# liyi14/mx-DeepIM

Measured on NVIDIA H100. Metric: 480x640 4-iter pose refinements/sec, higher is better.
Workload: dtype fp16

## Files before the change

mx-deepim_b200/csrc/conv_igemm.cuh:

```cuda
#pragma once
#include <cuda.h>
#include <cuda_fp16.h>
#include "common.cuh"
#include "wgmma.cuh"

namespace dim {

struct ConvKParams {
  CUtensorMap a_map[4];
  CUtensorMap a_lo_map[4];
  CUtensorMap b_map;
  CUtensorMap b_lo_map;
  CUtensorMap out_map[2];
  const __nv_bfloat16 *in_hi, *in_lo;
  int in_cols;
  int KH, KW, stride, cchunks;
  int BW, BH, n_col_tiles;
  int Hq, Ho, Wo, Bn;
  int out_Hp, out_Wp, out_py, out_px, Cout;
  int kblocks;
  float slope;
  const float *bias;
  __nv_bfloat16 *out_hi, *out_lo;
  int in_off_r, in_off_c;
// ... 127 lines not shown
}

__device__ __forceinline__ uint32_t pack2_f16(float a, float b) {
  uint32_t r;
  asm("cvt.rn.satfinite.f16x2.f32 %0, %1, %2;" : "=r"(r) : "f"(b), "f"(a));
  return r;
}
__device__ __forceinline__ uint32_t pack2_bf16(float a, float b) {
  uint32_t r;
  asm("cvt.rn.bf16x2.f32 %0, %1, %2;" : "=r"(r) : "f"(b), "f"(a));
  return r;
}

constexpr int kConv1Slack = 2048;


__device__ __forceinline__ int frag_row(int t) { return ((t >> 5) << 4) + ((t & 31) >> 2); }

__device__ __forceinline__ uint32_t pack2_bf16_lo(float v0, float v1, uint32_t hi) {
  return pack2_bf16(v0 - __uint_as_float(hi << 16), v1 - __uint_as_float(hi & 0xFFFF0000u));
}

template <bool SPLIT3, bool F16>
__device__ __forceinline__ void epi_pack(float v0, float v1, float b0, float b1, float slope, uint32_t &hi, uint32_t &lo) {
  v0 += b0;
  v1 += b1;
  v0 = v0 > 0.f ? v0 : v0 * slope;
  v1 = v1 > 0.f ? v1 : v1 * slope;
  if (F16) {
    hi = pack2_f16(v0, v1);
  } else {
    hi = pack2_bf16(v0, v1);
    if (SPLIT3) lo = pack2_bf16_lo(v0, v1, hi);
  }
}

template <bool SPLIT3, bool F16>
__device__ __forceinline__ void store_pair(float v0, float v1, float2 b, float slope, __nv_bfloat16 *out_hi, __nv_bfloat16 *out_lo,
                                           long long off) {
  uint32_t h, l = 0;
  epi_pack<SPLIT3, F16>(v0, v1, b.x, b.y, slope, h, l);
  *reinterpret_cast<uint32_t *>(out_hi + off) = h;
  if (SPLIT3) *reinterpret_cast<uint32_t *>(out_lo + off) = l;
}

template <bool SPLIT3>
__device__ __forceinline__ void store_pair_generic(float v0, float v1, const ConvKParams &p, int n, bool valid, long long off,
                                                   long long add_off, long long mask_off) {
  if (!valid || n >= p.Cout) return;
  if (p.bias) {
    v0 += __ldg(p.bias + n);
    v1 += __ldg(p.bias + n + 1);
  }
  if (p.addend.p) {
    const __nv_bfloat162 a = *reinterpret_cast<const __nv_bfloat162 *>(p.addend.p + add_off);
    if (SPLIT3) {
      const __nv_bfloat162 al = *reinterpret_cast<const __nv_bfloat162 *>(p.addend.lo + add_off);
      v0 += __low2float(a) + __low2float(al);
      v1 += __high2float(a) + __high2float(al);
    } else {
      v0 += __low2float(a);
      v1 += __high2float(a);
    }
  }
  if (p.mask.p) {
    if (n < p.mask_climit) {
      const __nv_bfloat162 m = *reinterpret_cast<const __nv_bfloat162 *>(p.mask.p + mask_off);
      if (!(__low2float(m) > 0.f)) v0 *= p.slope;
      if (!(__high2float(m) > 0.f)) v1 *= p.slope;
    }
  } else {
    v0 = v0 > 0.f ? v0 : v0 * p.slope;
    v1 = v1 > 0.f ? v1 : v1 * p.slope;
  }
  if (SPLIT3) {
    const uint32_t h = pack2_bf16(v0, v1);
    *reinterpret_cast<uint32_t *>(p.out_hi + off) = h;
    *reinterpret_cast<uint32_t *>(p.out_lo + off) = pack2_bf16_lo(v0, v1, h);
  } else {
    *reinterpret_cast<__nv_bfloat162 *>(p.out_hi + off) = __floats2bfloat162_rn(v0, v1);
  }
}

template <int BLOCK_N, int STAGES, bool SPLIT3, int EPI>
struct ConvSmem2 {
  static constexpr int A_BYTES = 128 * 64 * 2;
  static constexpr int B_BYTES = BLOCK_N * 64 * 2;
  static constexpr int NPREC = SPLIT3 ? 2 : 1;
  static constexpr int STAGE_BYTES = (A_BYTES + B_BYTES) * NPREC;
  static constexpr int RING_BYTES = STAGES * STAGE_BYTES;
  static constexpr int LIMIT = 227 * 1024, FIXED = 1024  + 256 ;
  static constexpr bool TMA_EPI = EPI == 0 && !SPLIT3;
  static constexpr int STG_GROUPS =
      !TMA_EPI ? 0 : (RING_BYTES + 2 * BLOCK_N * 128 + FIXED <= LIMIT ? BLOCK_N / 64 : BLOCK_N / 128);
  static constexpr int STG_ROUNDS = TMA_EPI ? BLOCK_N / 64 / STG_GROUPS : 0;
  static constexpr int STG_BYTES = STG_GROUPS * 8192;
  static constexpr int TOTAL = RING_BYTES + 2 * STG_BYTES + FIXED;
  static_assert(TOTAL <= LIMIT, "conv_igemm shared memory");
};

template <int BLOCK_N, int STAGES, bool SPLIT3, bool F16, int EPI = 0>
__global__ void __launch_bounds__(384, 1) conv_igemm_persistent_kernel(const __grid_constant__ ConvKParams p,
                                                                       const int total_tiles, const int n_tiles) {
  using S = ConvSmem2<BLOCK_N, STAGES, SPLIT3, EPI>;
  constexpr uint32_t SBO = 1024u;

  extern __shared__ uint8_t smem_raw[];
  uint8_t *smem = reinterpret_cast<uint8_t *>((reinterpret_cast<uintptr_t>(smem_raw) + 1023) & ~(uintptr_t)1023);
  uint8_t *stg = smem + S::RING_BYTES;
  uint64_t *full_bar = reinterpret_cast<uint64_t *>(stg + 2 * S::STG_BYTES);
  uint64_t *empty_bar = full_bar + STAGES;

  const int wgi = threadIdx.x >> 7, warp = threadIdx.x >> 5;

  if (threadIdx.x == 0) {
    for (int s = 0; s < STAGES; ++s) {
      ptx::mbar_init(&full_bar[s], 1);
      ptx::mbar_init(&empty_bar[s], 2);
    }
    ptx::fence_barrier_init();
    ptx::prefetch_tmap(&p.b_map);
    ptx::prefetch_tmap(&p.a_map[0]);
    if (S::TMA_EPI) ptx::prefetch_tmap(&p.out_map[0]);
  }
  __syncthreads();

  if (wgi == 0) {
    ptx::regs_producer();
    if (warp == 0) {
      const uint32_t tx = (uint32_t)(p.BW * p.BH * 64 * 2 + BLOCK_N * 64 * 2) * S::NPREC;
      int s = 0;
      uint32_t ph = 0;
      for (int tile = blockIdx.x; tile < total_tiles; tile += gridDim.x) {
        const int nt = tile % n_tiles, mt = tile / n_tiles;
        const int col_tile = mt % p.n_col_tiles, row_tile = mt / p.n_col_tiles;
        const int g0 = row_tile * p.BH, ow0 = col_tile * p.BW, n0 = nt * BLOCK_N;
        for (int kb = 0; kb < p.kblocks; ++kb) {
          ptx::mbar_wait(&empty_bar[s], ph ^ 1u);
          const int tap = kb / p.cchunks, cc = kb - tap * p.cchunks;
          const int kh = tap / p.KW, kw = tap - kh * p.KW;
          int view = 0, dr = kh, dc = kw;
          if (p.stride == 2) {
            view = ((kh & 1) << 1) | (kw & 1);
            dr = kh >> 1;
            dc = kw >> 1;
          }
          uint8_t *st = smem + s * S::STAGE_BYTES;
          if (EPI) { dr += p.in_off_r; dc += p.in_off_c; }
          if (ptx::elect_one()) {
            ptx::mbar_expect_tx_raw(&full_bar[s], tx);
            for (int pr = 0; pr < S::NPREC; ++pr) {
              uint8_t *sa = st + pr * (S::A_BYTES + S::B_BYTES);
              const CUtensorMap *am = pr ? &p.a_lo_map[view] : &p.a_map[view];
              ptx::tma_load_3d_raw(sa, am, &full_bar[s], cc * 64, ow0 + dc, g0 + dr);
              if (EPI == 0) ptx::tma_load_3d_raw(sa + S::A_BYTES / 2, am, &full_bar[s], cc * 64, ow0 + dc, g0 + dr + (p.BH >> 1));
              ptx::tma_load_2d_raw(sa + S::A_BYTES, pr ? &p.b_lo_map : &p.b_map, &full_bar[s], kb * 64, n0);
            }
          }
          __syncwarp();
          if (++s == STAGES) { s = 0; ph ^= 1u; }
        }
      }
    }
  } else {
    ptx::regs_consumer();
    const int t = threadIdx.x & 127;
    const int half = wgi - 1;
    const int q2 = (t & 3) * 2;
    const bool arriver = t == 0;
    const uint32_t base = ptx::smem_u32(smem);
    uint8_t *my_stg = stg + half * S::STG_BYTES;
    const int lane = t & 31;
    const uint32_t st_addr = ptx::smem_u32(my_stg) + (uint32_t)((16 * (t >> 5) + 8 * ((lane >> 3) & 1) + (lane & 7)) * 128);
    const uint32_t st_sw = (uint32_t)(((lane >> 4) & 1) ^ (lane & 7));
    float acc[BLOCK_N / 2];
    int s = 0;
    uint32_t ph = 0;
    for (int tile = blockIdx.x; tile < total_tiles; tile += gridDim.x) {
      int prev = -1;
      for (int kb = 0; kb < p.kblocks; ++kb) {
        ptx::mbar_wait(&full_bar[s], ph);
        const uint32_t a_hi = base + s * S::STAGE_BYTES + half * 8192;
        const uint32_t b_hi = base + s * S::STAGE_BYTES + S::A_BYTES;
        const uint64_t da0 = ptx::gmma_desc(a_hi, 16, SBO, ptx::kSW128), db0 = ptx::gmma_desc(b_hi, 16, SBO, ptx::kSW128);
        const uint64_t dal0 = da0 + ((S::A_BYTES + S::B_BYTES) >> 4), dbl0 = db0 + ((S::A_BYTES + S::B_BYTES) >> 4);
        wg::fence_acc(acc);
        wg::fence();
#pragma unroll
        for (int k = 0; k < 4; ++k) {
          const uint64_t da = da0 + (uint64_t)(2 * k), db = db0 + (uint64_t)(2 * k);
          wg::mma<BLOCK_N, F16, 0, 0>(acc, da, db, (kb > 0 || k > 0) ? 1u : 0u);
          if (SPLIT3) {
            wg::mma<BLOCK_N, false, 0, 0>(acc, dal0 + (uint64_t)(2 * k), db, 1u);
            wg::mma<BLOCK_N, false, 0, 0>(acc, da, dbl0 + (uint64_t)(2 * k), 1u);
          }
        }
        wg::commit();
        wg::wait<1>();
        wg::fence_acc(acc);
        if (prev >= 0 && arriver) ptx::mbar_arrive(&empty_bar[prev]);
        prev = s;
        if (++s == STAGES) { s = 0; ph ^= 1u; }
      }
      wg::wait<0>();
      wg::fence_acc(acc);
      if (prev >= 0 && arriver) ptx::mbar_arrive(&empty_bar[prev]);

      const int nt = tile % n_tiles, mt = tile / n_tiles;
      const int col_tile = mt % p.n_col_tiles, row_tile = mt / p.n_col_tiles;
      const int n0 = nt * BLOCK_N;
      if constexpr (S::TMA_EPI) {
        const int gs = row_tile * p.BH + half * (p.BH >> 1), ow0 = col_tile * p.BW;
        const int n_img = gs / p.Hq, oh = gs - n_img * p.Hq;
        const bool store0 = n_img < p.Bn && oh < p.Ho, store1 = n_img + 1 < p.Bn && oh + (p.BH >> 1) > p.Hq;
#pragma unroll
        for (int rd = 0; rd < S::STG_ROUNDS; ++rd) {
          if (arriver) ptx::bulk_wait_read0();
          ptx::named_bar_sync(1 + half, 128);
#pragma unroll
          for (int i = 0; i < S::STG_GROUPS * 4; ++i) {
            const int j = rd * S::STG_GROUPS * 8 + 2 * i;
            const float *bj = p.bias + n0 + 8 * j + q2;
            const float b0 = __ldg(bj), b1 = __ldg(bj + 1), b2 = __ldg(bj + 8), b3 = __ldg(bj + 9);
            uint32_t h[4], unused;
            epi_pack<false, F16>(acc[4 * j + 0], acc[4 * j + 1], b0, b1, p.slope, h[0], unused);
            epi_pack<false, F16>(acc[4 * j + 2], acc[4 * j + 3], b0, b1, p.slope, h[1], unused);
            epi_pack<false, F16>(acc[4 * j + 4], acc[4 * j + 5], b2, b3, p.slope, h[2], unused);
            epi_pack<false, F16>(acc[4 * j + 6], acc[4 * j + 7], b2, b3, p.slope, h[3], unused);
            ptx::stmatrix_x4(st_addr + (uint32_t)((i >> 2) * 8192) + (((uint32_t)(2 * (i & 3)) ^ st_sw) << 4), h);
          }
          ptx::fence_proxy_async();
          ptx::named_bar_sync(1 + half, 128);
          if (arriver && store0) {
            for (int q = 0; q < S::STG_GROUPS; ++q)
              ptx::tma_store_4d(&p.out_map[0], my_stg + q * 8192, n0 + (rd * S::STG_GROUPS + q) * 64, ow0, oh, n_img);
            ptx::bulk_commit();
          }
        }
        if (store1) {
#pragma unroll
          for (int rr = 0; rr < 2; ++rr) {
            const int lr = frag_row(t) + rr * 8, bh = lr / p.BW;
            const int oh1 = oh + bh - p.Hq, ow = ow0 + lr - bh * p.BW;
            if (lr < p.BW * (p.BH >> 1) && oh1 >= 0 && oh1 < p.Ho) {
              const long long off =
                  (((long long)(n_img + 1) * p.out_Hp + oh1 + p.out_py) * p.out_Wp + ow + p.out_px) * p.Cout + n0 + q2;
#pragma unroll
              for (int j = 0; j < BLOCK_N / 8; ++j)
                store_pair<false, F16>(acc[4 * j + 2 * rr], acc[4 * j + 2 * rr + 1],
                                       make_float2(__ldg(p.bias + n0 + 8 * j + q2), __ldg(p.bias + n0 + 8 * j + q2 + 1)), p.slope,
                                       p.out_hi, p.out_lo, off + 8 * j);
            }
          }
        }
      } else {
#pragma unroll
        for (int rr = 0; rr < 2; ++rr) {
          const int lr = frag_row(t) + rr * 8, m = EPI ? half * 64 + lr : lr;
          const bool in_tile = EPI ? m < p.BW * p.BH : lr < p.BW * (p.BH >> 1);
          const int bh = m / p.BW, bw = m - bh * p.BW;
          const int g = row_tile * p.BH + (EPI ? 0 : half * (p.BH >> 1)) + bh, ow = col_tile * p.BW + bw;
          const int n_img = g / p.Hq, oh = g - n_img * p.Hq;
          if (EPI == 1) {
            const int y = oh * p.out_sy + p.out_oy, x = ow * p.out_sx + p.out_ox;
            const bool valid = in_tile && (n_img < p.Bn) && (oh < p.Ho) && (ow < p.Wo) && y >= 0 && y < p.out_H &&
                               x >= 0 && x < p.out_W;
            const long long off =
                (((long long)n_img * p.out_Hp + y + p.out_py) * p.out_Wp + x + p.out_px) * p.out_cs + p.out_coff + n0 + q2;
            const long long add_off =
                (((long long)n_img * p.addend.Hp + y + p.addend.py) * p.addend.Wp + x + p.addend.px) * p.addend.cs + p.addend.coff +
                n0 + q2;
            const long long mask_off =
                (((long long)n_img * p.mask.Hp + y + p.mask.py) * p.mask.Wp + x + p.mask.px) * p.mask.cs + p.mask.coff + n0 + q2;
#pragma unroll
            for (int j = 0; j < BLOCK_N / 8; ++j)
              store_pair_generic<SPLIT3>(acc[4 * j + 2 * rr], acc[4 * j + 2 * rr + 1], p, n0 + 8 * j + q2, valid, off + 8 * j,
                                 add_off + 8 * j, mask_off + 8 * j);
          } else {
            const bool valid = in_tile && (n_img < p.Bn) && (oh < p.Ho) && (ow < p.Wo);
            if (valid) {
              const long long off = (((long long)n_img * p.out_Hp + oh + p.out_py) * p.out_Wp + ow + p.out_px) * p.Cout + n0 + q2;
#pragma unroll
              for (int j = 0; j < BLOCK_N / 8; ++j)
                store_pair<SPLIT3, F16>(acc[4 * j + 2 * rr], acc[4 * j + 2 * rr + 1],
                                        make_float2(__ldg(p.bias + n0 + 8 * j + q2), __ldg(p.bias + n0 + 8 * j + q2 + 1)), p.slope, p.out_hi,
                                        p.out_lo, off + 8 * j);
            }
          }
        }
      }
    }
    if (S::TMA_EPI && arriver) ptx::bulk_wait0();
  }
}

constexpr int kConv1StoreN = 80;

template <int N, int STAGES, bool SPLIT3>
struct Conv1Smem {
  static constexpr int NPREC = SPLIT3 ? 2 : 1;
  static constexpr int TAP_BYTES = 64 * 32 * 2;
  static constexpr int RES_BYTES = 16 * TAP_BYTES * NPREC;
  static constexpr int STG_BYTES = N * 128;
  static constexpr int PLANE_BYTES = (N + 3) * 16;
  static constexpr int STRIP_BYTES = (4 * PLANE_BYTES + 127) / 128 * 128;
  static constexpr int STAGE_BYTES = STRIP_BYTES * NPREC;
  static constexpr int TOTAL = RES_BYTES + 2 * STG_BYTES * NPREC + STAGES * STAGE_BYTES + 1024  + 256 ;
  static_assert(N % kConv1StoreN == 0 && N % 16 == 0 && STG_BYTES % 1024 == 0, "conv1 tile width");
  static_assert(TOTAL <= 227 * 1024, "conv1 shared memory");
};

template <int N, int STAGES, bool SPLIT3, bool F16>
__global__ void __launch_bounds__(384, 1) conv1_kernel(const __grid_constant__ ConvKParams p, const int rows_total,
                                                       const int rows_per_chunk, const int chunks_per_col) {
  using S = Conv1Smem<N, STAGES, SPLIT3>;
  extern __shared__ uint8_t smem_raw[];
  uint8_t *smem = reinterpret_cast<uint8_t *>((reinterpret_cast<uintptr_t>(smem_raw) + 1023) & ~(uintptr_t)1023);
  uint8_t *res = smem;
  uint8_t *stg = res + S::RES_BYTES;
  uint8_t *ring = stg + 2 * S::NPREC * S::STG_BYTES;
  uint64_t *full_bar = reinterpret_cast<uint64_t *>(ring + STAGES * S::STAGE_BYTES);
  uint64_t *empty_bar = full_bar + STAGES;
  uint64_t *res_bar = empty_bar + STAGES;

  const int wgi = threadIdx.x >> 7, warp = threadIdx.x >> 5;
  const int ct = blockIdx.x / chunks_per_col, ck = blockIdx.x - ct * chunks_per_col;
  const int g_lo = ck * rows_per_chunk;
  const int g_hi = min(rows_total, g_lo + rows_per_chunk);
  const int n_rows = max(0, g_hi - g_lo);
  const int n_strips = n_rows > 0 ? n_rows + 3 : 0;
  const int ow0 = ct * N;

  if (threadIdx.x == 0) {
    for (int s = 0; s < STAGES; ++s) {
      ptx::mbar_init(&full_bar[s], 1);
      ptx::mbar_init(&empty_bar[s], 2);
    }
    ptx::mbar_init(res_bar, 1);
    ptx::fence_barrier_init();
    ptx::prefetch_tmap(&p.b_map);
    ptx::prefetch_tmap(&p.out_map[0]);
  }
  __syncthreads();

  if (wgi == 0) {
    ptx::regs_producer();
    if (warp == 0 && n_rows > 0) {
      if (ptx::elect_one()) {
        ptx::mbar_expect_tx_raw(res_bar, (uint32_t)S::RES_BYTES);
        for (int kb = 0; kb < 16; ++kb) {
          ptx::tma_load_2d_raw(res + kb * S::TAP_BYTES, &p.b_map, res_bar, kb * 32, 0);
          if (SPLIT3) ptx::tma_load_2d_raw(res + (16 + kb) * S::TAP_BYTES, &p.b_lo_map, res_bar, kb * 32, 0);
        }
      }
      __syncwarp();
      const size_t plane = (size_t)p.in_cols * 16;
      const uint8_t *src_hi = reinterpret_cast<const uint8_t *>(p.in_hi) + (size_t)ow0 * 16;
      const uint8_t *src_lo = reinterpret_cast<const uint8_t *>(p.in_lo) + (size_t)ow0 * 16;
      for (int s = 0; s < n_strips; ++s) {
        const int slot = s % STAGES;
        ptx::mbar_wait(&empty_bar[slot], (((uint32_t)(s / STAGES)) & 1u) ^ 1u);
        uint8_t *st = ring + slot * S::STAGE_BYTES;
        if (g_lo + s >= rows_total) {
          if (ptx::elect_one()) ptx::mbar_arrive(&full_bar[slot]);
        } else if (ptx::elect_one()) {
          ptx::mbar_expect_tx_raw(&full_bar[slot], (uint32_t)(4 * S::PLANE_BYTES * S::NPREC));
          const size_t row = (size_t)(g_lo + s) * 4 * plane;
#pragma unroll
          for (int c = 0; c < 4; ++c) {
            ptx::bulk_load_raw(st + c * S::PLANE_BYTES, src_hi + row + c * plane, S::PLANE_BYTES, &full_bar[slot]);
            if (SPLIT3)
              ptx::bulk_load_raw(st + S::STRIP_BYTES + c * S::PLANE_BYTES, src_lo + row + c * plane, S::PLANE_BYTES, &full_bar[slot]);
          }
        }
        __syncwarp();
// ... 230 lines not shown
```

mx-deepim_b200/csrc/net.cu:

```cuda
#include <cuda_fp16.h>
#include <string.h>

#include <memory>
#include <mutex>

#include "launch.cuh"
#include "net_state.cuh"

namespace dim {

static void build_geometry(NetState *ns, int H, int W) {
  int h = H, w = W;
  for (int i = 0; i < 10; ++i) {
    const LayerSpec &s = kLayers[i];
    LayerGeom &g = ns->g[i];
    g.Cin = s.Cin; g.Cout = s.Cout; g.k = s.k; g.stride = s.stride; g.pad = s.pad;
    g.Hin = h; g.Win = w;
    g.Ho = (h + 2 * s.pad - s.k) / s.stride + 1;
    g.Wo = (w + 2 * s.pad - s.k) / s.stride + 1;
    if (g.Ho < 1) g.Ho = 1;
    if (g.Wo < 1) g.Wo = 1;
    int Hp = h + 2 * s.pad, Wp = w + 2 * s.pad;
    if (s.stride == 2) { Hp += Hp & 1; Wp += Wp & 1; }
    g.py = g.px = s.pad;
// ... 395 lines not shown
    DIM_LAUNCH_CHECK();
  }
  pack_fc6_kernel<<<256 * FC6_K / 256, 256, 0, st>>>(w[10], ns->fc6_w_hi, L(ns->fc6_w_lo), F(ns->fc6_w_f16));
  DIM_LAUNCH_CHECK();
  transpose256_kernel<<<256, 256, 0, st>>>(w[11], ns->fc7_wT);
  DIM_LAUNCH_CHECK();
  ns->lo_stale = !with_lo;
  ns->f16_stale = !with_f16;
  return 0;
}

__global__ void __launch_bounds__(256) f16_from_hilo_kernel(const __nv_bfloat16 *hi, const __nv_bfloat16 *lo, size_t n,
                                                            __nv_bfloat16 *out) {
  const size_t i = (size_t)blockIdx.x * blockDim.x + threadIdx.x;
  if (i >= n) return;
  const __half h = __float2half_rn(__bfloat162float(hi[i]) + __bfloat162float(lo[i]));
  reinterpret_cast<__half *>(out)[i] = h;
}

static int net_refresh_f16(dim_ctx *ctx, cudaStream_t st) {
  NetState *ns = ctx->net;
  if (ns->lo_stale)
    if (int rc = train_refresh_lo(ctx, st)) return rc;
  for (int i = 0; i < 10; ++i) {
    const LayerGeom &g = ns->g[i];
    const size_t n = (size_t)g.Cout * g.KH * g.KW * g.Ceff;
    f16_from_hilo_kernel<<<(unsigned)((n + 255) / 256), 256, 0, st>>>(ns->w_hi[i], ns->w_lo[i], n, ns->w_f16[i]);
    DIM_LAUNCH_CHECK();
  }
  const size_t n6 = (size_t)256 * FC6_K;
  f16_from_hilo_kernel<<<(unsigned)((n6 + 255) / 256), 256, 0, st>>>(ns->fc6_w_hi, ns->fc6_w_lo, n6, ns->fc6_w_f16);
  DIM_LAUNCH_CHECK();
  ns->f16_stale = false;
  return 0;
}

int net_load(dim_ctx *ctx, const float *const *W, const float *const *Bv) {
  NetState *ns = ctx->net;
  DIM_REQUIRE(ns != nullptr, "net not created");
  DIM_REQUIRE(ns->net_ok, "dim_net_load: FlowNetS + fc6 (81920 inputs) needs a 480x640 context");
  DIM_REQUIRE(!ns->train_aliased, "dim_net_load: this context trains; use dim_train_load_params (it owns the weights)");
  if (ns->loaded) DIM_CHECK(cudaDeviceSynchronize());
  if (int rc = net_alloc_weights(ctx)) return rc;
  size_t n[12], off[13] = {0};
  for (int i = 0; i < 10; ++i) {
    const LayerGeom &g = ns->g[i];
    const int cin = i == 0 && !ns->input_depth ? (ns->input_mask ? 8 : 6) : g.Cin;
    n[i] = (size_t)g.Cout * cin * g.k * g.k;
  }
  n[10] = (size_t)256 * FC6_K;
  n[11] = 256 * 256;
  for (int i = 0; i < 12; ++i) off[i + 1] = off[i] + n[i];
  float *stage_p = nullptr;
  DIM_CHECK(cudaMalloc(&stage_p, off[12] * sizeof(float)));
  std::unique_ptr<float, cudaError_t (*)(void *)> stage(stage_p, cudaFree);
  auto put = [](float *dst, const float *src, size_t count) {
    return cudaMemcpy(dst, src, count * sizeof(float), cudaMemcpyHostToDevice);
  };
  const float *w[12];
  for (int i = 0; i < 12; ++i) {
    w[i] = stage.get() + off[i];
    if (i != 10) DIM_CHECK(put(stage.get() + off[i], W[i], n[i]));
  }
  {
    std::vector<float> p((size_t)256 * FC6_K);
    for (int o = 0; o < 256; ++o)
      for (int c = 0; c < 1024; ++c)
        for (int hw = 0; hw < 80; ++hw) p[(size_t)o * FC6_K + (size_t)hw * 1024 + c] = W[10][(size_t)o * FC6_K + (size_t)c * 80 + hw];
    DIM_CHECK(put(stage.get() + off[10], p.data(), n[10]));
  }
  for (int i = 0; i < 10; ++i) DIM_CHECK(put(ns->bias[i], Bv[i], ns->g[i].Cout));
  DIM_CHECK(put(ns->fc6_b, Bv[10], 256));
  DIM_CHECK(put(ns->fc7_b, Bv[11], 256));
  DIM_CHECK(put(ns->rot_w, W[12], 4 * 256));
  DIM_CHECK(put(ns->rot_b, Bv[12], 4));
  DIM_CHECK(put(ns->trans_w, W[13], 3 * 256));
  DIM_CHECK(put(ns->trans_b, Bv[13], 3));
  if (int rc = net_pack_weights(ctx, w, 0, true, true)) return rc;
  DIM_CHECK(cudaStreamSynchronize(0));
  ns->loaded = true;
  return 0;
}

template <int BN, int ST, bool S3, bool F16>
static int launch_conv(const ConvKParams &kp, int total_tiles, int n_tiles, int cap, cudaStream_t st) {
  using S = ConvSmem2<BN, ST, S3, 0>;
  static bool attr_set = false;
  if (!attr_set) {
    DIM_CHECK(cudaFuncSetAttribute(conv_igemm_persistent_kernel<BN, ST, S3, F16>, cudaFuncAttributeMaxDynamicSharedMemorySize,
                                   S::TOTAL));
    attr_set = true;
  }
  const int grid = total_tiles < cap ? total_tiles : cap;
  conv_igemm_persistent_kernel<BN, ST, S3, F16><<<grid, 384, S::TOTAL, st>>>(kp, total_tiles, n_tiles);
  DIM_LAUNCH_CHECK();
  return 0;
}

template <int N, int ST, bool S3, bool F16>
static int launch_conv1(const ConvKParams &kp, int grid, int rows_total, int rpc, int chunks, cudaStream_t st) {
  using S = Conv1Smem<N, ST, S3>;
  static bool set = false;
  if (!set) {
    DIM_CHECK(cudaFuncSetAttribute(conv1_kernel<N, ST, S3, F16>, cudaFuncAttributeMaxDynamicSharedMemorySize, S::TOTAL));
    set = true;
  }
  conv1_kernel<N, ST, S3, F16><<<grid, 384, S::TOTAL, st>>>(kp, rows_total, rpc, chunks);
  DIM_LAUNCH_CHECK();
  return 0;
}

template <int ST, bool S3, bool F16, int NB>
static int launch_conv1_rgbd(const ConvKParams &kp, int grid, int rows_total, int rpc, int chunks, int strip_bytes,
                             cudaStream_t st) {
  const int smem_bytes = 16 * NB * 128 * (S3 ? 2 : 1) + ST * (S3 ? 2 : 1) * strip_bytes + kConv1Slack + 1024 + 256;
  DIM_REQUIRE(smem_bytes <= 227 * 1024, "conv1 (RGB-D): image too wide for the rolling-strip ring");
  static int set = 0;
  if (set < smem_bytes) {
    DIM_CHECK(cudaFuncSetAttribute(conv1_rgbd_kernel<ST, S3, F16, NB>, cudaFuncAttributeMaxDynamicSharedMemorySize,
                                   smem_bytes));
    set = smem_bytes;
  }
  conv1_rgbd_kernel<ST, S3, F16, NB><<<grid, 384, smem_bytes, st>>>(kp, rows_total, rpc, chunks, strip_bytes);
  DIM_LAUNCH_CHECK();
  return 0;
}

int net_set_input_depth(dim_ctx *ctx, bool enable) {
  NetState *ns = ctx->net;
  DIM_REQUIRE(ns != nullptr, "net not created");
  if (ns->input_depth == enable) return 0;
  DIM_REQUIRE(!ns->loaded, "dim_ctx_set_input_depth: call it before dim_net_load (this context's weights are loaded)");
  if (!ns->act0_rgb_hi) { ns->act0_rgb_hi = ns->act_hi[0]; ns->act0_rgb_lo = ns->act_lo[0]; }
  ns->input_depth = enable;
  build_geometry(ns, ctx->H, ctx->W);
  ns->maps.clear();
  const LayerGeom &g = ns->g[0];
  const size_t per = (size_t)g.rows * g.cols * g.Cbuf;
  ns->act_elems_per_image[0] = per;
  if (enable && ns->net_ok && !ns->act0_rgbd_hi) {
    if (int rc = dev_alloc(ctx, &ns->act0_rgbd_hi, per * ctx->max_batch, true)) return rc;
    if (int rc = dev_alloc(ctx, &ns->act0_rgbd_lo, per * ctx->max_batch, true)) return rc;
  }
  ns->act_hi[0] = enable ? ns->act0_rgbd_hi : ns->act0_rgb_hi;
  ns->act_lo[0] = enable ? ns->act0_rgbd_lo : ns->act0_rgb_lo;
  return 0;
}

bool net_input_depth(dim_ctx *ctx) { return ctx->net && ctx->net->input_depth; }

int net_set_input_mask(dim_ctx *ctx, bool enable) {
  NetState *ns = ctx->net;
  DIM_REQUIRE(ns != nullptr, "net not created");
  if (ns->input_mask == enable) return 0;
  DIM_REQUIRE(!ns->loaded, "dim_ctx_set_input_mask: call it before dim_net_load (this context's weights are loaded)");
  ns->input_mask = enable;
  return 0;
}

bool net_input_mask(dim_ctx *ctx) { return !ctx->net || ctx->net->input_mask; }

void net_input_geometry(dim_ctx *ctx, int *rows, int *cols, int *pad, __nv_bfloat16 **hi, __nv_bfloat16 **lo) {
  NetState *ns = ctx->net;
  *rows = ns->g[0].rows; *cols = ns->g[0].cols; *pad = ns->g[0].py;
  *hi = ns->act_hi[0]; *lo = ns->act_lo[0];
}

int net_forward(dim_ctx *ctx, int B, int precision, const float *zoom_factor, float *rot_out, float *trans_out,
                float *se3_out, cudaStream_t st, cudaEvent_t after_conv) {
  NetState *ns = ctx->net;
  DIM_REQUIRE(ns && ns->loaded, "dim_net_load has not been called");
  DIM_REQUIRE(B >= 1 && B <= ctx->max_batch, "batch exceeds max_batch");
  DIM_REQUIRE(precision == DIM_PREC_BF16 || precision == DIM_PREC_BF16X3 || precision == DIM_PREC_FP16,
              "unknown precision (DIM_PREC_BF16 / DIM_PREC_BF16X3 / DIM_PREC_FP16)");
  const bool s3 = precision == DIM_PREC_BF16X3, f16 = precision == DIM_PREC_FP16;
  const int key = B + (f16 ? kF16MapKey : 0);
  auto it = ns->maps.find(key);
  if (it == ns->maps.end()) {
    TensorMaps tm;
    if (int rc = build_maps(ns, B, f16, tm)) return rc;
    it = ns->maps.emplace(key, tm).first;
  }
  const TensorMaps &tm = it->second;
  if (ns->repack_done) DIM_CHECK(cudaStreamWaitEvent(st, ns->repack_done, 0));
  if (s3 && ns->lo_stale)
    if (int rc = train_refresh_lo(ctx, st)) return rc;
  if (f16 && ns->f16_stale)
    if (int rc = net_refresh_f16(ctx, st)) return rc;
  if (ns->layer_events) DIM_CHECK(cudaEventRecord(ns->layer_events[0], st));
  for (int i = 0; i < 10; ++i) {
    const LayerGeom &g = ns->g[i];
    const ConvKParams &kp = tm.kp[i];
    const int n_tiles = g.Cout / g.BLOCK_N;
    const int total_tiles = cdiv(B * g.Hq, g.BH) * g.n_col_tiles * n_tiles;
    const int sms = ns->num_sms;
    int rc;
    if (i == 0 && ns->input_depth) {
      const int nsplit = s3 ? 4 : 1;
      const int rows_total = B * g.Hq;
      int chunks = sms / (g.n_col_tiles * nsplit);
      if (chunks > cdiv(rows_total, 16)) chunks = cdiv(rows_total, 16);
      if (chunks < 1) chunks = 1;
      const int rpc = cdiv(rows_total, chunks);
      chunks = cdiv(rows_total, rpc);
      const int strip_bytes = cdiv((g.BW + 3) * 128, 128) * 128;
      const int grid = g.n_col_tiles * chunks * nsplit;
      rc = s3 ? launch_conv1_rgbd<5, true, false, 16>(kp, grid, rows_total, rpc, chunks, strip_bytes, st)
              : (f16 ? launch_conv1_rgbd<6, false, true, 64>(kp, grid, rows_total, rpc, chunks, strip_bytes, st)
                     : launch_conv1_rgbd<6, false, false, 64>(kp, grid, rows_total, rpc, chunks, strip_bytes, st));
    } else if (i == 0) {
      DIM_REQUIRE(g.Wo == 320 && g.cols >= g.Wo + 3 && g.Hq == g.rows && g.Hq == g.Ho + 3,
                  "conv1_kernel is built for a 480x640 input (320 output columns)");
      const int n_col = g.Wo / (s3 ? 80 : 160);
      const int rows_total = B * g.Hq;
      int chunks = sms / n_col;
      if (chunks > cdiv(rows_total, 16)) chunks = cdiv(rows_total, 16);
      if (chunks < 1) chunks = 1;
      const int rpc = cdiv(rows_total, chunks);
      chunks = cdiv(rows_total, rpc);
      const int grid = n_col * chunks;
      rc = s3 ? launch_conv1<80, 5, true, false>(kp, grid, rows_total, rpc, chunks, st)
              : (f16 ? launch_conv1<160, 8, false, true>(kp, grid, rows_total, rpc, chunks, st)
                     : launch_conv1<160, 8, false, false>(kp, grid, rows_total, rpc, chunks, st));
    } else if (g.BLOCK_N == 128) {
      rc = s3 ? launch_conv<128, 3, true, false>(kp, total_tiles, n_tiles, sms, st)
              : (f16 ? launch_conv<128, 6, false, true>(kp, total_tiles, n_tiles, sms, st)
                     : launch_conv<128, 6, false, false>(kp, total_tiles, n_tiles, sms, st));
    } else {
      rc = s3 ? launch_conv<256, 2, true, false>(kp, total_tiles, n_tiles, sms, st)
              : (f16 ? launch_conv<256, 4, false, true>(kp, total_tiles, n_tiles, sms, st)
                     : launch_conv<256, 4, false, false>(kp, total_tiles, n_tiles, sms, st));
    }
    if (rc) return rc;
    if (ns->layer_events && i < 9) DIM_CHECK(cudaEventRecord(ns->layer_events[i + 1], st));
  }
  if (ns->layer_events) DIM_CHECK(cudaEventRecord(ns->layer_events[10], st));
  if (after_conv) DIM_CHECK(cudaEventRecord(after_conv, st));
  if (s3)
    fc6_mma_kernel<true><<<FC6_SPLITS, 256, 0, st>>>(ns->act_hi[10], ns->act_lo[10], ns->fc6_w_hi, ns->fc6_w_lo, B,
                                                     ctx->max_batch, ns->fc6_partial);
  else if (f16)
    fc6_mma_kernel<false, true><<<FC6_SPLITS, 256, 0, st>>>(ns->act_hi[10], nullptr, ns->fc6_w_f16, nullptr, B,
                                                            ctx->max_batch, ns->fc6_partial);
  else
    fc6_mma_kernel<false><<<FC6_SPLITS, 256, 0, st>>>(ns->act_hi[10], nullptr, ns->fc6_w_hi, nullptr, B,
                                                      ctx->max_batch, ns->fc6_partial);
  DIM_LAUNCH_CHECK();
  head_kernel<<<B, 1024, 0, st>>>(ns->fc6_partial, ctx->max_batch, ns->fc6_b, ns->fc7_wT, ns->fc7_b, ns->rot_w,
                                 ns->rot_b, ns->trans_w, ns->trans_b, zoom_factor, rot_out, trans_out, se3_out, ns->save_h6,
                                 ns->save_h7);
  DIM_LAUNCH_CHECK();
  return 0;
}

bool net_graph_safe(dim_ctx *ctx) {
  NetState *ns = ctx->net;
  return ns && ns->loaded && !ns->layer_events && !ns->train_aliased;
}

int net_layer_profile(dim_ctx *ctx, int enable, float *ms10) {
  NetState *ns = ctx->net;
  DIM_REQUIRE(ns != nullptr, "net not created");
  if (enable && !ns->layer_events) {
    ns->layer_events = new cudaEvent_t[11];
    for (int i = 0; i < 11; ++i) DIM_CHECK(cudaEventCreate(&ns->layer_events[i]));
  }
  if (ms10 && ns->layer_events) {
    DIM_CHECK(cudaDeviceSynchronize());
    for (int i = 0; i < 10; ++i) DIM_CHECK(cudaEventElapsedTime(&ms10[i], ns->layer_events[i], ns->layer_events[i + 1]));
  }
  if (!enable && ns->layer_events) {
    for (int i = 0; i < 11; ++i) cudaEventDestroy(ns->layer_events[i]);
    delete[] ns->layer_events;
    ns->layer_events = nullptr;
  }
  return 0;
}

int net_debug_activation(dim_ctx *ctx, int idx, int lo, void *host_dst, size_t bytes) {
  NetState *ns = ctx->net;
  DIM_REQUIRE(ns && idx >= 0 && idx <= 10, "bad activation index");
  const size_t have = ns->act_elems_per_image[idx] * ctx->max_batch * 2;
  DIM_REQUIRE(bytes <= have, "activation copy larger than buffer");
  DIM_CHECK(cudaMemcpy(host_dst, lo ? ns->act_lo[idx] : ns->act_hi[idx], bytes, cudaMemcpyDeviceToHost));
  return 0;
}

void net_layer_geometry(dim_ctx *ctx, int idx, int *out ) {
  NetState *ns = ctx->net;
  if (idx < 10) {
    const LayerGeom &g = ns->g[idx];
    out[0] = g.rows; out[1] = g.cols; out[2] = g.Cbuf; out[3] = g.py; out[4] = g.px; out[5] = g.Ho; out[6] = g.Wo;
    out[7] = g.Cout;
  } else {
    const LayerGeom &g = ns->g[9];
    out[0] = g.Ho; out[1] = g.Wo; out[2] = g.Cout; out[3] = 0; out[4] = 0; out[5] = 0; out[6] = 0; out[7] = 256;
  }
}

}
```

Measured before the change: 3289.

## Use 256-pixel M tiles for N=128 convs and defer epilogue into next tile's mainloop

For the BLOCK_N=128 fp16/bf16 conv layers, each consumer warpgroup now holds two 64-row accumulators, so a tile covers 256 output pixels and every B tile loaded is reused across twice as many pixels. The pipeline drops from 6 to 4 stages to fit the larger A stage. The TMA-store epilogue is packed into registers and deferred: its staging and store rounds are issued during the first k-blocks of the next tile, so stores overlap the MMAs. The cost is higher register pressure, fewer tiles (and so possibly worse SM balance on small layers), and a shallower pipeline.

Measured after the change: 3351, median of 6. 1.02x the previous value.

```diff
diff --git a/mx-deepim_b200/csrc/conv_igemm.cuh b/mx-deepim_b200/csrc/conv_igemm.cuh
--- a/mx-deepim_b200/csrc/conv_igemm.cuh
+++ b/mx-deepim_b200/csrc/conv_igemm.cuh
@@ -233,9 +233,10 @@
   }
 }
 
-template <int BLOCK_N, int STAGES, bool SPLIT3, int EPI>
+template <int BLOCK_N, int STAGES, bool SPLIT3, int EPI, int MSUB = 1>
 struct ConvSmem2 {
-  static constexpr int A_BYTES = 128 * 64 * 2;
+  static_assert(MSUB == 1 || (MSUB == 2 && EPI == 0 && !SPLIT3 && BLOCK_N == 128), "256-pixel tiles: fp16 / bf16 forward, N = 128");
+  static constexpr int A_BYTES = MSUB * 128 * 64 * 2;
   static constexpr int B_BYTES = BLOCK_N * 64 * 2;
   static constexpr int NPREC = SPLIT3 ? 2 : 1;
   static constexpr int STAGE_BYTES = (A_BYTES + B_BYTES) * NPREC;
@@ -244,16 +245,17 @@
   static constexpr bool TMA_EPI = EPI == 0 && !SPLIT3;
   static constexpr int STG_GROUPS =
       !TMA_EPI ? 0 : (RING_BYTES + 2 * BLOCK_N * 128 + FIXED <= LIMIT ? BLOCK_N / 64 : BLOCK_N / 128);
-  static constexpr int STG_ROUNDS = TMA_EPI ? BLOCK_N / 64 / STG_GROUPS : 0;
+  static constexpr int SUB_ROUNDS = TMA_EPI ? BLOCK_N / 64 / STG_GROUPS : 1;
+  static constexpr int STG_ROUNDS = TMA_EPI ? MSUB * SUB_ROUNDS : 0;
   static constexpr int STG_BYTES = STG_GROUPS * 8192;
   static constexpr int TOTAL = RING_BYTES + 2 * STG_BYTES + FIXED;
   static_assert(TOTAL <= LIMIT, "conv_igemm shared memory");
 };
 
-template <int BLOCK_N, int STAGES, bool SPLIT3, bool F16, int EPI = 0>
+template <int BLOCK_N, int STAGES, bool SPLIT3, bool F16, int EPI = 0, int MSUB = 1>
 __global__ void __launch_bounds__(384, 1) conv_igemm_persistent_kernel(const __grid_constant__ ConvKParams p,
                                                                        const int total_tiles, const int n_tiles) {
-  using S = ConvSmem2<BLOCK_N, STAGES, SPLIT3, EPI>;
+  using S = ConvSmem2<BLOCK_N, STAGES, SPLIT3, EPI, MSUB>;
   constexpr uint32_t SBO = 1024u;
 
   extern __shared__ uint8_t smem_raw[];
@@ -279,13 +281,13 @@
   if (wgi == 0) {
     ptx::regs_producer();
     if (warp == 0) {
-      const uint32_t tx = (uint32_t)(p.BW * p.BH * 64 * 2 + BLOCK_N * 64 * 2) * S::NPREC;
+      const uint32_t tx = (uint32_t)(MSUB * p.BW * p.BH * 64 * 2 + BLOCK_N * 64 * 2) * S::NPREC;
       int s = 0;
       uint32_t ph = 0;
       for (int tile = blockIdx.x; tile < total_tiles; tile += gridDim.x) {
         const int nt = tile % n_tiles, mt = tile / n_tiles;
         const int col_tile = mt % p.n_col_tiles, row_tile = mt / p.n_col_tiles;
-        const int g0 = row_tile * p.BH, ow0 = col_tile * p.BW, n0 = nt * BLOCK_N;
+        const int g0 = row_tile * p.BH * MSUB, ow0 = col_tile * p.BW, n0 = nt * BLOCK_N;
         for (int kb = 0; kb < p.kblocks; ++kb) {
           ptx::mbar_wait(&empty_bar[s], ph ^ 1u);
           const int tap = kb / p.cchunks, cc = kb - tap * p.cchunks;
@@ -303,8 +305,12 @@
             for (int pr = 0; pr < S::NPREC; ++pr) {
               uint8_t *sa = st + pr * (S::A_BYTES + S::B_BYTES);
               const CUtensorMap *am = pr ? &p.a_lo_map[view] : &p.a_map[view];
-              ptx::tma_load_3d_raw(sa, am, &full_bar[s], cc * 64, ow0 + dc, g0 + dr);
-              if (EPI == 0) ptx::tma_load_3d_raw(sa + S::A_BYTES / 2, am, &full_bar[s], cc * 64, ow0 + dc, g0 + dr + (p.BH >> 1));
+              if (EPI == 0) {
+                for (int q = 0; q < 2 * MSUB; ++q)
+                  ptx::tma_load_3d_raw(sa + q * 8192, am, &full_bar[s], cc * 64, ow0 + dc, g0 + dr + q * (p.BH >> 1));
+              } else {
+                ptx::tma_load_3d_raw(sa, am, &full_bar[s], cc * 64, ow0 + dc, g0 + dr);
+              }
               ptx::tma_load_2d_raw(sa + S::A_BYTES, pr ? &p.b_lo_map : &p.b_map, &full_bar[s], kb * 64, n0);
             }
           }
@@ -324,86 +330,101 @@
     const int lane = t & 31;
     const uint32_t st_addr = ptx::smem_u32(my_stg) + (uint32_t)((16 * (t >> 5) + 8 * ((lane >> 3) & 1) + (lane & 7)) * 128);
     const uint32_t st_sw = (uint32_t)(((lane >> 4) & 1) ^ (lane & 7));
-    float acc[BLOCK_N / 2];
+    float acc[MSUB][BLOCK_N / 2];
+    constexpr int kEpiRound1Kb = 4;
+    uint32_t pk[MSUB][BLOCK_N / 4];
+    int e_n0 = 0, e_ow0 = 0, e_g0 = 0;
+    auto epi_round = [&](const int rd) {
+      const int m = rd / S::SUB_ROUNDS, c = rd - m * S::SUB_ROUNDS;
+      const int gs = e_g0 + m * (p.BH >> 1), n_img = gs / p.Hq, oh = gs - n_img * p.Hq;
+      if (arriver) ptx::bulk_wait_read0();
+      ptx::named_bar_sync(1 + half, 128);
+#pragma unroll
+      for (int i = 0; i < S::STG_GROUPS * 4; ++i) {
+        const int j = c * S::STG_GROUPS * 8 + 2 * i;
+        const uint32_t h[4] = {pk[m][2 * j], pk[m][2 * j + 1], pk[m][2 * j + 2], pk[m][2 * j + 3]};
+        ptx::stmatrix_x4(st_addr + (uint32_t)((i >> 2) * 8192) + (((uint32_t)(2 * (i & 3)) ^ st_sw) << 4), h);
+      }
+      ptx::fence_proxy_async();
+      ptx::named_bar_sync(1 + half, 128);
+      if (arriver && n_img < p.Bn && oh < p.Ho) {
+        for (int q = 0; q < S::STG_GROUPS; ++q)
+          ptx::tma_store_4d(&p.out_map[0], my_stg + q * 8192, e_n0 + (c * S::STG_GROUPS + q) * 64, e_ow0, oh, n_img);
+        ptx::bulk_commit();
+      }
+      if (c == S::SUB_ROUNDS - 1 && n_img + 1 < p.Bn && oh + (p.BH >> 1) > p.Hq) {
+#pragma unroll
+        for (int rr = 0; rr < 2; ++rr) {
+          const int lr = frag_row(t) + rr * 8, bh = lr / p.BW;
+          const int oh1 = oh + bh - p.Hq, ow = e_ow0 + lr - bh * p.BW;
+          if (lr < p.BW * (p.BH >> 1) && oh1 >= 0 && oh1 < p.Ho) {
+            const long long off =
+                (((long long)(n_img + 1) * p.out_Hp + oh1 + p.out_py) * p.out_Wp + ow + p.out_px) * p.Cout + e_n0 + q2;
+#pragma unroll
+            for (int j = 0; j < BLOCK_N / 8; ++j) *reinterpret_cast<uint32_t *>(p.out_hi + off + 8 * j) = pk[m][2 * j + rr];
+          }
+        }
+      }
+    };
     int s = 0;
     uint32_t ph = 0;
     for (int tile = blockIdx.x; tile < total_tiles; tile += gridDim.x) {
+      const bool deferred = S::TMA_EPI && tile != blockIdx.x;
       int prev = -1;
       for (int kb = 0; kb < p.kblocks; ++kb) {
         ptx::mbar_wait(&full_bar[s], ph);
-        const uint32_t a_hi = base + s * S::STAGE_BYTES + half * 8192;
+        const uint32_t a_hi = base + s * S::STAGE_BYTES + MSUB * half * 8192;
         const uint32_t b_hi = base + s * S::STAGE_BYTES + S::A_BYTES;
         const uint64_t da0 = ptx::gmma_desc(a_hi, 16, SBO, ptx::kSW128), db0 = ptx::gmma_desc(b_hi, 16, SBO, ptx::kSW128);
         const uint64_t dal0 = da0 + ((S::A_BYTES + S::B_BYTES) >> 4), dbl0 = db0 + ((S::A_BYTES + S::B_BYTES) >> 4);
-        wg::fence_acc(acc);
+#pragma unroll
+        for (int m = 0; m < MSUB; ++m) wg::fence_acc(acc[m]);
         wg::fence();
 #pragma unroll
         for (int k = 0; k < 4; ++k) {
           const uint64_t da = da0 + (uint64_t)(2 * k), db = db0 + (uint64_t)(2 * k);
-          wg::mma<BLOCK_N, F16, 0, 0>(acc, da, db, (kb > 0 || k > 0) ? 1u : 0u);
+#pragma unroll
+          for (int m = 0; m < MSUB; ++m)
+            wg::mma<BLOCK_N, F16, 0, 0>(acc[m], da + (uint64_t)(m * (8192 >> 4)), db, (kb > 0 || k > 0) ? 1u : 0u);
           if (SPLIT3) {
-            wg::mma<BLOCK_N, false, 0, 0>(acc, dal0 + (uint64_t)(2 * k), db, 1u);
-            wg::mma<BLOCK_N, false, 0, 0>(acc, da, dbl0 + (uint64_t)(2 * k), 1u);
+            wg::mma<BLOCK_N, false, 0, 0>(acc[0], dal0 + (uint64_t)(2 * k), db, 1u);
+            wg::mma<BLOCK_N, false, 0, 0>(acc[0], da, dbl0 + (uint64_t)(2 * k), 1u);
           }
         }
         wg::commit();
+        if (deferred) {
+          if (kb == 0) epi_round(0);
+          if constexpr (S::STG_ROUNDS > 1)
+            if (kb == min(kEpiRound1Kb, p.kblocks - 1)) epi_round(1);
+        }
         wg::wait<1>();
-        wg::fence_acc(acc);
+#pragma unroll
+        for (int m = 0; m < MSUB; ++m) wg::fence_acc(acc[m]);
         if (prev >= 0 && arriver) ptx::mbar_arrive(&empty_bar[prev]);
         prev = s;
         if (++s == STAGES) { s = 0; ph ^= 1u; }
       }
       wg::wait<0>();
-      wg::fence_acc(acc);
+#pragma unroll
+      for (int m = 0; m < MSUB; ++m) wg::fence_acc(acc[m]);
       if (prev >= 0 && arriver) ptx::mbar_arrive(&empty_bar[prev]);
 
       const int nt = tile % n_tiles, mt = tile / n_tiles;
       const int col_tile = mt % p.n_col_tiles, row_tile = mt / p.n_col_tiles;
       const int n0 = nt * BLOCK_N;
       if constexpr (S::TMA_EPI) {
-        const int gs = row_tile * p.BH + half * (p.BH >> 1), ow0 = col_tile * p.BW;
-        const int n_img = gs / p.Hq, oh = gs - n_img * p.Hq;
-        const bool store0 = n_img < p.Bn && oh < p.Ho, store1 = n_img + 1 < p.Bn && oh + (p.BH >> 1) > p.Hq;
-#pragma unroll
-        for (int rd = 0; rd < S::STG_ROUNDS; ++rd) {
-          if (arriver) ptx::bulk_wait_read0();
-          ptx::named_bar_sync(1 + half, 128);
-#pragma unroll
-          for (int i = 0; i < S::STG_GROUPS * 4; ++i) {
-            const int j = rd * S::STG_GROUPS * 8 + 2 * i;
-            const float *bj = p.bias + n0 + 8 * j + q2;
-            const float b0 = __ldg(bj), b1 = __ldg(bj + 1), b2 = __ldg(bj + 8), b3 = __ldg(bj + 9);
-            uint32_t h[4], unused;
-            epi_pack<false, F16>(acc[4 * j + 0], acc[4 * j + 1], b0, b1, p.slope, h[0], unused);
-            epi_pack<false, F16>(acc[4 * j + 2], acc[4 * j + 3], b0, b1, p.slope, h[1], unused);
-            epi_pack<false, F16>(acc[4 * j + 4], acc[4 * j + 5], b2, b3, p.slope, h[2], unused);
-            epi_pack<false, F16>(acc[4 * j + 6], acc[4 * j + 7], b2, b3, p.slope, h[3], unused);
-            ptx::stmatrix_x4(st_addr + (uint32_t)((i >> 2) * 8192) + (((uint32_t)(2 * (i & 3)) ^ st_sw) << 4), h);
-          }
-          ptx::fence_proxy_async();
-          ptx::named_bar_sync(1 + half, 128);
-          if (arriver && store0) {
-            for (int q = 0; q < S::STG_GROUPS; ++q)
-              ptx::tma_store_4d(&p.out_map[0], my_stg + q * 8192, n0 + (rd * S::STG_GROUPS + q) * 64, ow0, oh, n_img);
-            ptx::bulk_commit();
-          }
-        }
-        if (store1) {
-#pragma unroll
-          for (int rr = 0; rr < 2; ++rr) {
-            const int lr = frag_row(t) + rr * 8, bh = lr / p.BW;
-            const int oh1 = oh + bh - p.Hq, ow = ow0 + lr - bh * p.BW;
-            if (lr < p.BW * (p.BH >> 1) && oh1 >= 0 && oh1 < p.Ho) {
-              const long long off =
-                  (((long long)(n_img + 1) * p.out_Hp + oh1 + p.out_py) * p.out_Wp + ow + p.out_px) * p.Cout + n0 + q2;
-#pragma unroll
-              for (int j = 0; j < BLOCK_N / 8; ++j)
-                store_pair<false, F16>(acc[4 * j + 2 * rr], acc[4 * j + 2 * rr + 1],
-                                       make_float2(__ldg(p.bias + n0 + 8 * j + q2), __ldg(p.bias + n0 + 8 * j + q2 + 1)), p.slope,
-                                       p.out_hi, p.out_lo, off + 8 * j);
-            }
-          }
-        }
+        e_n0 = n0;
+        e_ow0 = col_tile * p.BW;
+        e_g0 = (row_tile * MSUB * 2 + MSUB * half) * (p.BH >> 1);
+#pragma unroll
+        for (int m = 0; m < MSUB; ++m)
+#pragma unroll
+          for (int j = 0; j < BLOCK_N / 8; ++j) {
+            const float b0 = __ldg(p.bias + n0 + 8 * j + q2), b1 = __ldg(p.bias + n0 + 8 * j + q2 + 1);
+            uint32_t unused;
+            epi_pack<false, F16>(acc[m][4 * j + 0], acc[m][4 * j + 1], b0, b1, p.slope, pk[m][2 * j], unused);
+            epi_pack<false, F16>(acc[m][4 * j + 2], acc[m][4 * j + 3], b0, b1, p.slope, pk[m][2 * j + 1], unused);
+          }
       } else {
 #pragma unroll
         for (int rr = 0; rr < 2; ++rr) {
@@ -425,7 +446,7 @@
                 (((long long)n_img * p.mask.Hp + y + p.mask.py) * p.mask.Wp + x + p.mask.px) * p.mask.cs + p.mask.coff + n0 + q2;
 #pragma unroll
             for (int j = 0; j < BLOCK_N / 8; ++j)
-              store_pair_generic<SPLIT3>(acc[4 * j + 2 * rr], acc[4 * j + 2 * rr + 1], p, n0 + 8 * j + q2, valid, off + 8 * j,
+              store_pair_generic<SPLIT3>(acc[0][4 * j + 2 * rr], acc[0][4 * j + 2 * rr + 1], p, n0 + 8 * j + q2, valid, off + 8 * j,
                                  add_off + 8 * j, mask_off + 8 * j);
           } else {
             const bool valid = in_tile && (n_img < p.Bn) && (oh < p.Ho) && (ow < p.Wo);
@@ -433,7 +454,7 @@
               const long long off = (((long long)n_img * p.out_Hp + oh + p.out_py) * p.out_Wp + ow + p.out_px) * p.Cout + n0 + q2;
 #pragma unroll
               for (int j = 0; j < BLOCK_N / 8; ++j)
-                store_pair<SPLIT3, F16>(acc[4 * j + 2 * rr], acc[4 * j + 2 * rr + 1],
+                store_pair<SPLIT3, F16>(acc[0][4 * j + 2 * rr], acc[0][4 * j + 2 * rr + 1],
                                         make_float2(__ldg(p.bias + n0 + 8 * j + q2), __ldg(p.bias + n0 + 8 * j + q2 + 1)), p.slope, p.out_hi,
                                         p.out_lo, off + 8 * j);
             }
@@ -441,7 +462,11 @@
         }
       }
     }
-    if (S::TMA_EPI && arriver) ptx::bulk_wait0();
+    if constexpr (S::TMA_EPI) {
+#pragma unroll
+      for (int rd = 0; rd < S::STG_ROUNDS; ++rd) epi_round(rd);
+      if (arriver) ptx::bulk_wait0();
+    }
   }
 }
 
diff --git a/mx-deepim_b200/csrc/net.cu b/mx-deepim_b200/csrc/net.cu
--- a/mx-deepim_b200/csrc/net.cu
+++ b/mx-deepim_b200/csrc/net.cu
@@ -501,17 +501,19 @@
   return 0;
 }
 
-template <int BN, int ST, bool S3, bool F16>
-static int launch_conv(const ConvKParams &kp, int total_tiles, int n_tiles, int cap, cudaStream_t st) {
-  using S = ConvSmem2<BN, ST, S3, 0>;
+template <int BN, int ST, bool S3, bool F16, int MSUB = 1>
+static int launch_conv(const ConvKParams &kp, const LayerGeom &g, int B, int cap, cudaStream_t st) {
+  using S = ConvSmem2<BN, ST, S3, 0, MSUB>;
   static bool attr_set = false;
   if (!attr_set) {
-    DIM_CHECK(cudaFuncSetAttribute(conv_igemm_persistent_kernel<BN, ST, S3, F16>, cudaFuncAttributeMaxDynamicSharedMemorySize,
-                                   S::TOTAL));
+    DIM_CHECK(cudaFuncSetAttribute(conv_igemm_persistent_kernel<BN, ST, S3, F16, 0, MSUB>,
+                                   cudaFuncAttributeMaxDynamicSharedMemorySize, S::TOTAL));
     attr_set = true;
   }
+  const int n_tiles = g.Cout / BN;
+  const int total_tiles = cdiv(B * g.Hq, g.BH * MSUB) * g.n_col_tiles * n_tiles;
   const int grid = total_tiles < cap ? total_tiles : cap;
-  conv_igemm_persistent_kernel<BN, ST, S3, F16><<<grid, 384, S::TOTAL, st>>>(kp, total_tiles, n_tiles);
+  conv_igemm_persistent_kernel<BN, ST, S3, F16, 0, MSUB><<<grid, 384, S::TOTAL, st>>>(kp, total_tiles, n_tiles);
   DIM_LAUNCH_CHECK();
   return 0;
 }
@@ -610,8 +612,6 @@
   for (int i = 0; i < 10; ++i) {
     const LayerGeom &g = ns->g[i];
     const ConvKParams &kp = tm.kp[i];
-    const int n_tiles = g.Cout / g.BLOCK_N;
-    const int total_tiles = cdiv(B * g.Hq, g.BH) * g.n_col_tiles * n_tiles;
     const int sms = ns->num_sms;
     int rc;
     if (i == 0 && ns->input_depth) {
@@ -642,13 +642,13 @@
               : (f16 ? launch_conv1<160, 8, false, true>(kp, grid, rows_total, rpc, chunks, st)
                      : launch_conv1<160, 8, false, false>(kp, grid, rows_total, rpc, chunks, st));
     } else if (g.BLOCK_N == 128) {
-      rc = s3 ? launch_conv<128, 3, true, false>(kp, total_tiles, n_tiles, sms, st)
-              : (f16 ? launch_conv<128, 6, false, true>(kp, total_tiles, n_tiles, sms, st)
-                     : launch_conv<128, 6, false, false>(kp, total_tiles, n_tiles, sms, st));
+      rc = s3 ? launch_conv<128, 3, true, false>(kp, g, B, sms, st)
+              : (f16 ? launch_conv<128, 4, false, true, 2>(kp, g, B, sms, st)
+                     : launch_conv<128, 4, false, false, 2>(kp, g, B, sms, st));
     } else {
-      rc = s3 ? launch_conv<256, 2, true, false>(kp, total_tiles, n_tiles, sms, st)
-              : (f16 ? launch_conv<256, 4, false, true>(kp, total_tiles, n_tiles, sms, st)
-                     : launch_conv<256, 4, false, false>(kp, total_tiles, n_tiles, sms, st));
+      rc = s3 ? launch_conv<256, 2, true, false>(kp, g, B, sms, st)
+              : (f16 ? launch_conv<256, 4, false, true>(kp, g, B, sms, st)
+                     : launch_conv<256, 4, false, false>(kp, g, B, sms, st));
     }
     if (rc) return rc;
     if (ns->layer_events && i < 9) DIM_CHECK(cudaEventRecord(ns->layer_events[i + 1], st));
```
